# Wenlin-Chen/ADKF-IFT

Hardware: AMD Instinct MI355X
Metric: meta-tasks/sec (N_support=128, d=256) (higher is better)
Workload: dtype f32

## Files before the change

### adkf_ift_amd/csrc/adkf_gp.hip

```cpp
#include <hip/hip_runtime.h>
#include <algorithm>
#include <cstdio>
#include <cstdlib>

#include "../../include/adkf_gp.h"
#include "ard.h"
#include "pna.h"
#include "readout.h"
#include "block.h"
#include "outer_step.h"
#include "refine64.h"
#include "hyper.h"
#include "large_fused.h"
#include "gemm_x3.h"
#include "dense_x3.h"
#include "predict_stream.h"
#include "thompson_stream.h"

using namespace adkf;

namespace {

constexpr int MAX_POINTS = 4096;
constexpr int REG_POINTS = 128;
// ... 362 lines not shown

Refine64Args refine_args(const TaskView& tv, const adkf_batch_t* b, const Workspace& w, bool with_hessian, int level, float* f_out,
                         int32_t* info, float* f_in, float* g_in, float* gnorm, size_t& lds_bytes) {
    const bool lds_inv = refine64_lds_optin();
    lds_bytes = lds_inv ? sizeof(double) * (size_t)R64_LDS_POINTS * R64_LDS_POINTS : 0;
    return Refine64Args{tv, b->Z_s, b->Z_q, b->d, b->y_s, b->y_q, b->priors, w.Ainv, with_hessian ? w.P : nullptr, level >= 1 ? w.C : nullptr,
                        level >= 2 ? w.S : nullptr, w.vecs, w.scal, f_out, info, f_in, g_in, gnorm, w.w64, w.w64_stride, r64_threshold(), b->T,
                        with_hessian ? 1 : 0, level, lds_inv ? 1 : 0};
}

void launch_refine(const TaskView& tv, const adkf_batch_t* b, const Workspace& w, bool with_hessian, int level, float* f_out,
                   int32_t* info, hipStream_t st, float* f_in = nullptr, float* g_in = nullptr, float* gnorm = nullptr) {
    if (!w.w64) return;
    size_t lds_bytes;
    const Refine64Args ra = refine_args(tv, b, w, with_hessian, level, f_out, info, f_in, g_in, gnorm, lds_bytes);
    k_refine64<<<b->T, R64_NT, lds_bytes, st>>>(ra);
}

bool use_fused_outer(int ns, int nq) {
    static const bool enabled = [] { const char* e = getenv("ADKF_FUSED_OUTER"); return !e || atoi(e) != 0; }();
    static const bool optin = [] {
        bool ok = true;
        for (const void* f : {reinterpret_cast<const void*>(&k_hyper<true, 0>), reinterpret_cast<const void*>(&k_hyper<true, 1>),
                              reinterpret_cast<const void*>(&k_hyper<false, 0>), reinterpret_cast<const void*>(&k_hyper<false, 1>)})
            ok = ok && hipFuncSetAttribute(f, hipFuncAttributeMaxDynamicSharedMemorySize, (int)HY_LDS_BYTES) == hipSuccess;
        return ok;
    }();
    if (!optin) (void)hipGetLastError();
    const int hi = ns > nq ? ns : nq;
    return enabled && optin && hi >= 1 && hi <= HY_N;
}

int launch_outer_factor(const OuterArgs& a, const Workspace& w, int nq, hipStream_t st) {
    if (nq > REG_POINTS) {
        k_lg_resid<<<dim3(ceil_div(nq, 4), a.T), 256, 0, st>>>(a);
        LgMat m = lg_mat(w, a.S, a.tv.nq_ld, a.tv.n_q, nullptr, a.T);
        lg_sweep(m, st);
        LgMatvecArgs mv{m, a.vecs + (size_t)V_R * a.tv.vld, (size_t)NVEC * a.tv.vld, a.vecs + (size_t)V_E * a.tv.vld, (size_t)NVEC * a.tv.vld, -1.f};
        k_lg_matvec<<<dim3(ceil_div(nq, 4), a.T), 256, 0, st>>>(mv);
        const int tn = ceil_div(nq, GT);
        k_lg_negate<<<grid_for(a.T, tn * tn), 256, 0, st>>>(m, tn);
        LgColsumArgs cs{a.C, a.tv.ns_ld, (size_t)a.tv.nq_ld * a.tv.ns_ld, a.tv.n_q, a.tv.nq_ld, a.tv.n_s, a.tv.ns_ld,
                        a.vecs + (size_t)V_E * a.tv.vld, (size_t)NVEC * a.tv.vld, a.vecs + (size_t)V_CTE * a.tv.vld, (size_t)NVEC * a.tv.vld};
        k_lg_colsum<<<dim3(ceil_div(a.tv.ns_ld, 64), a.T), 1024, 0, st>>>(cs);
        LgOuterFin fin{a, w.lg_logdet, w.lg_info, w.lg_pext};
        k_lg_outer_fin<<<a.T, 64, 0, st>>>(fin);
        LAUNCH_OK();
        return 0;
    }
    if (nq <= 16) k_outer_factor<16, 256><<<grid_for(a.T, 1), 256, 0, st>>>(a);
    else if (nq <= 32) k_outer_factor<32, 256><<<grid_for(a.T, 1), 256, 0, st>>>(a);
    else if (nq <= 64) k_outer_factor<64, 256><<<grid_for(a.T, 1), 256, 0, st>>>(a);
    else k_outer_factor<128, 512><<<grid_for(a.T, 1), 512, 0, st>>>(a);
    LAUNCH_OK();
    return 0;
}


InnerArgs inner_args(const adkf_batch_t* b, const Workspace& w, float* phi, int32_t* info) {
    InnerArgs a{};
    a.D2ss = w.D2ss; a.y_s = b->y_s; a.n_s = b->n_s; a.phi = phi; a.priors = b->priors;
    a.Ainv = w.Ainv; a.vecs = w.vecs; a.scal = w.scal; a.info = info;
    a.T = b->T; a.ld = b->ns_max; a.vld = w.vld; a.kind = b->kernel;
    a.max_evals = 0; a.exact_evals = 0; a.gtol = 0.f; a.ftol = 0.f;
    return a;
}

int outer_pipeline(const adkf_batch_t* b, const Workspace& w, const float* phi, int flags, bool with_hessian, float* f_out,
                   float* dZ_s, float* dZ_q, float* g_phi_out, float* v_out, float* H_out, int32_t* info, hipStream_t st) {
    const int T = b->T, ns = b->ns_max, nq = b->nq_max, d = b->d;
    int rc = stage_dist(b, w, true, st);
    if (rc) return rc;
    const bool reuse_inner = (b->flags & ADKF_BATCH_REUSE_INNER) != 0;
    if (!reuse_inner) {
        InnerArgs ia = inner_args(b, w, const_cast<float*>(phi), info);
        rc = launch_inner(ia, w, st);
        if (rc) return rc;
    }
    TaskView tv = make_tv(b, w, true);
    const int tms = ceil_div(ns, GT), tmq = ceil_div(nq, GT);
    const float dirscale = (flags & ADKF_IGNORE_DIRECT_GRAD) ? 0.f : 1.f;
    const float corrscale = (with_hessian && !(flags & ADKF_IGNORE_GRAD_CORRECTION)) ? 1.f : 0.f;
    if (use_fused_outer(ns, nq)) {
        HyperArgs ha{tv, w.Ainv, w.D2ss, w.D2qs, w.D2qq, b->y_s, b->y_q, b->priors, w.Wss, w.Wqs, w.Wqq, w.P, w.OC, w.S, w.vecs, w.scal, f_out, info,
                     g_phi_out, v_out, H_out, T, reuse_inner ? 1 : 0, with_hessian ? 1 : 0, flags, dirscale, corrscale, refine32_threshold()};
        const bool full = ns == HY_N && nq == HY_N && !b->n_s && !b->n_q && tv.vec;
        const bool rbf = b->kernel == ADKF_KERNEL_RBF;
        if (full && rbf) k_hyper<true, 0><<<grid_for(T, 1), HY_NT, HY_LDS_BYTES, st>>>(ha);
        else if (full) k_hyper<true, 1><<<grid_for(T, 1), HY_NT, HY_LDS_BYTES, st>>>(ha);
        else if (rbf) k_hyper<false, 0><<<grid_for(T, 1), HY_NT, HY_LDS_BYTES, st>>>(ha);
        else k_hyper<false, 1><<<grid_for(T, 1), HY_NT, HY_LDS_BYTES, st>>>(ha);
    } else {
    launch_alpha_refine(tv, b, w, st);
    if (with_hessian) {
        ProbP pp; pp.tv = tv; pp.Ainv = w.Ainv; pp.D2ss = w.D2ss; pp.P = w.P;
        launch_gemm(pp, T, ns, ns, st);
        HessArgs ha{tv, w.Ainv, w.P, w.D2ss, b->y_s, b->priors, w.scal, w.vecs, T};
        if (ns > REG_POINTS) {
            k_lg_hess_mv<<<dim3(ceil_div(ns, 4), T), 256, 0, st>>>(ha);
            LgMat am = lg_mat(w, w.Ainv, ns, b->n_s, nullptr, T);
            LgMatvecArgs mv{am, w.vecs + (size_t)V_BETA * w.vld, (size_t)NVEC * w.vld, w.vecs + (size_t)V_DELTA * w.vld, (size_t)NVEC * w.vld, 1.f};
            k_lg_matvec<<<dim3(ceil_div(ns, 4), T), 256, 0, st>>>(mv);
            LgHessTr ht{ha, w.lg_part, tms * tms, tms};
            k_lg_hess_tr<<<grid_for(T, tms * tms), 256, 0, st>>>(ht);
            k_lg_hess_fin<<<T, 64, 0, st>>>(ht);
        } else {
            k_hess<<<grid_for(T, 1), SMALL_NT, 0, st>>>(ha);
        }
    }
    launch_c(tv, b, w, st);
    ProbS ps; ps.tv = tv; ps.C = w.C; ps.D2qs = w.D2qs; ps.D2qq = w.D2qq; ps.S = w.S;
    launch_gemm(ps, T, nq, nq, st);
    OuterArgs oa{tv, w.C, w.S, b->y_s, b->y_q, w.vecs, w.scal, f_out, info, T, reuse_inner ? 1 : 0};
    rc = launch_outer_factor(oa, w, nq, st);
    if (rc) return rc;
    ProbOC po; po.tv = tv; po.Sinv = w.S; po.C = w.C; po.D2qs = w.D2qs; po.OC = w.OC; po.Wqs = w.Wqs; po.part = w.part_oc; po.ntiles = w.nt_oc; po.dirscale = dirscale;
    launch_gemm(po, T, nq, ns, st);
    ProbMA pm; pm.tv = tv; pm.C = w.C; pm.OC = w.OC; pm.D2ss = w.D2ss; pm.Wss = w.Wss; pm.part = w.part_ma; pm.ntiles = w.nt_ma; pm.dirscale = dirscale;
    launch_gemm(pm, T, ns, ns, st);
    SolveArgs sa{tv, w.scal, w.vecs, w.part_oc, w.part_ma, w.nt_oc, w.nt_ma, flags, g_phi_out, v_out, H_out, T, with_hessian ? 1 : 0};
    WqqArgs wq{tv, w.S, w.D2qq, w.Wqq, w.scal, dirscale, T, 0, sa};
    if (nq > REG_POINTS) {
        LgWqq lw{wq, w.lg_part, tmq * tmq, tmq};
        k_lg_wqq<<<grid_for(T, tmq * tmq), 256, 0, st>>>(lw);
        k_lg_wqq_fin<<<T, 64, 0, st>>>(lw);
        k_solve_v<<<T, 64, 0, st>>>(sa);
    } else {
        wq.do_solve = 1;
        k_wqq<<<grid_for(T, 1), SMALL_NT, 0, st>>>(wq);
    }
    if (corrscale != 0.f) {
        ProbMixed px; px.tv = tv; px.Ainv = w.Ainv; px.P = w.P; px.D2ss = w.D2ss; px.Wss = w.Wss; px.corrscale = corrscale;
        launch_gemm(px, T, ns, ns, st);
    }
    }
    if (dZ_s || dZ_q) {
        if (dZ_s && b->n_s) hipMemsetAsync(dZ_s, 0, (size_t)T * ns * d * sizeof(float), st);
        if (dZ_q && b->n_q) hipMemsetAsync(dZ_q, 0, (size_t)T * nq * d * sizeof(float), st);
        ProbDZ<false> pzs; pzs.tv = tv; pzs.Wss = w.Wss; pzs.Wqs = w.Wqs; pzs.Wqq = w.Wqq; pzs.Zs = b->Z_s; pzs.Zq = b->Z_q; pzs.dZ = dZ_s; pzs.d = d;
        ProbDZ<true> pzq; pzq.tv = tv; pzq.Wss = w.Wss; pzq.Wqs = w.Wqs; pzq.Wqq = w.Wqq; pzq.Zs = b->Z_s; pzq.Zq = b->Z_q; pzq.dZ = dZ_q; pzq.d = d;
        if (dZ_s) launch_gemm(pzs, T, ns, d, st, x3_for(d));
        if (dZ_q) launch_gemm(pzq, T, nq, d, st, x3_for(d));
    }
    if (w.w64) {
        size_t lds_bytes;
        const Refine64Args ra = refine_args(tv, b, w, with_hessian, 2, f_out, info, nullptr, nullptr, nullptr, lds_bytes);
        Cot64Args ca{tv, b->Z_s, b->Z_q, dZ_s, dZ_q, d, w.vecs, w.scal, w.w64, w.w64_stride, r64_threshold(), T,
                     with_hessian ? 1 : 0, flags, dirscale, corrscale, g_phi_out, v_out, H_out, lds_bytes ? 1 : 0};
        k_tail64<<<T, R64_NT, lds_bytes, st>>>(ra, ca);
    }
    LAUNCH_OK();
    return 0;
}


struct ArdWs {
    float *mu, *ell, *Zt_s, *Zt_q, *G, *Gd_s, *Gd_q, *Gdot, *phi3, *pri3, *f3, *g3, *g3o, *S1, *gt, *coldot;
    float *c, *ut2, *wn, *Ddot, *Wdot, *adot, *S2;
    ArdFitState* fst; float *x, *g, *p, *xe, *ge, *S, *Y, *fe; int32_t* info3;
    ArdCgState* cst; float *cx, *cr, *cp, *cHp, *gout; int32_t* n_eff;
    size_t bytes;
};

ArdWs carve_ard(void* base, size_t off0, int T, int ns, int nq, int d) {
    ArdWs a;
    size_t off = off0;
    auto take = [&](size_t nfloat) { float* p = base ? reinterpret_cast<float*>(static_cast<char*>(base) + off) : nullptr; off += align_up((nfloat ? nfloat : 1) * sizeof(float)); return p; };
// ... 1208 lines not shown
```

### adkf_ift_amd/csrc/hyper.h

```cpp
#pragma once
#include "kernels.h"

namespace adkf {

constexpr int HY_NT = 512, HY_N = 128;
constexpr int HY_LDK = 132;
constexpr int HY_LDM = 144;
constexpr int HY_BUF = HY_N * HY_LDM;
constexpr int HY_NVEC = 10;
constexpr int HY_LDS_FLOATS = 2 * HY_BUF + HY_NVEC * HY_N + 9 * (HY_NT / 64) + 8;
constexpr size_t HY_LDS_BYTES = sizeof(float) * HY_LDS_FLOATS;

struct HyperArgs {
    TaskView tv;
    const float *Ainv, *D2ss, *D2qs, *D2qq, *y_s, *y_q, *priors;
    float *Wss, *Wqs, *Wqq;
    float *stash_ss, *stash_qs, *stash_qq;
    float* vecs; float* scal; float* f_out; int32_t* info;
    float *g_phi_out, *v_out, *H_out;
    int T, reset_info, with_hessian, flags;
    float dirscale, corrscale, refine_thresh;
};

__device__ __forceinline__ float hy_ex(int kind, float u) { return kind == 0 ? expf(-0.5f * u) : expf(-SQRT5 * sqrtf(u)); }
__device__ __forceinline__ float hy_k0(int kind, float u, float ex) { return kind == 0 ? ex : (1.f + SQRT5 * sqrtf(u) + (5.f / 3.f) * u) * ex; }
__device__ __forceinline__ float hy_ex_of_k0(int kind, float u, float k0) { return kind == 0 ? k0 : k0 / (1.f + SQRT5 * sqrtf(u) + (5.f / 3.f) * u); }
__device__ __forceinline__ void hy_k3(int kind, float u, float ex, float& k0, float& k1, float& k2) {
    if (kind == 0) { k0 = ex; k1 = -0.5f * ex; k2 = 0.25f * ex; }
    else {
        const float r = sqrtf(u);
        k0 = (1.f + SQRT5 * r + (5.f / 3.f) * u) * ex;
        k1 = -(5.f / 6.f) * (1.f + SQRT5 * r) * ex;
        k2 = (25.f / 12.f) * ex;
    }
}

#define HY_OPAQUE1(v_) asm volatile("" : "+v"(v_))
__device__ __forceinline__ int hy_tid() { int t = threadIdx.x; HY_OPAQUE1(t); return t; }
template <bool FULL>
__device__ __forceinline__ void hy_fetch(float4 (&v)[8], const float* src, int src_ld, int rows) {
    const int tid = threadIdx.x;
    unsigned base = (unsigned)((tid >> 5) * HY_N + (tid & 31) * 4);
    if (FULL) HY_OPAQUE1(base);
#pragma unroll
    for (int u = 0; u < 8; ++u) {
        const int r = (tid >> 5) + 16 * u, c4 = (tid & 31) * 4;
        if (FULL) v[u] = *reinterpret_cast<const float4*>(src + (base + 16u * u * HY_N));
        else {
            const int rc = r < rows ? r : rows - 1, cc = c4 + 3 < src_ld ? c4 : 0;
            v[u] = *reinterpret_cast<const float4*>(src + (unsigned)(rc * src_ld + cc));
        }
    }
}
template <bool FULL, class F>
__device__ __forceinline__ void hy_put(float* buf, int ld, const float4 (&v)[8], int rows, int cols, F f) {
    const int tid = hy_tid();
#pragma unroll
    for (int u = 0; u < 8; ++u) {
        const int r = (tid >> 5) + 16 * u, c4 = (tid & 31) * 4;
        float4 o;
        o.x = (FULL || (r < rows && c4 + 0 < cols)) ? f(v[u].x, r, c4 + 0) : 0.f;
        o.y = (FULL || (r < rows && c4 + 1 < cols)) ? f(v[u].y, r, c4 + 1) : 0.f;
        o.z = (FULL || (r < rows && c4 + 2 < cols)) ? f(v[u].z, r, c4 + 2) : 0.f;
        o.w = (FULL || (r < rows && c4 + 3 < cols)) ? f(v[u].w, r, c4 + 3) : 0.f;
        *reinterpret_cast<float4*>(buf + r * ld + c4) = o;
    }
}
template <bool FULL, class F>
__device__ __forceinline__ void hy_load(float* buf, int ld, const float* src, int src_ld, int rows, int cols, bool vec, F f) {
    if (FULL || vec) {
        float4 v[8];
        hy_fetch<FULL>(v, src, src_ld, rows);
        hy_put<FULL>(buf, ld, v, rows, cols, f);
    } else {
        for (int e = threadIdx.x; e < HY_N * HY_N; e += HY_NT) {
            const int r = e >> 7, c = e & 127;
            buf[r * ld + c] = (r < rows && c < cols) ? f(src[(unsigned)(r * src_ld + c)], r, c) : 0.f;
        }
    }
}

template <bool FULL, bool SYM>
__device__ __forceinline__ void hy_dist(float (&dv)[8][4], const float* D, int ld, int rows, int cols) {
    const int lane = threadIdx.x & 63, p = lane & 15, g = lane >> 4, w = threadIdx.x >> 6;
    if (FULL && SYM) {
        unsigned q = (unsigned)(p * HY_N + 16 * w + 4 * g);
        HY_OPAQUE1(q);
#pragma unroll
        for (int x = 0; x < 8; ++x) {
            const float4 t = *reinterpret_cast<const float4*>(D + (q + 16u * x * HY_N));
            dv[x][0] = t.x; dv[x][1] = t.y; dv[x][2] = t.z; dv[x][3] = t.w;
        }
    } else if (FULL) {
        unsigned q = (unsigned)((16 * w + 4 * g) * HY_N + p);
        HY_OPAQUE1(q);
#pragma unroll
        for (int x = 0; x < 8; ++x)
#pragma unroll
            for (int y = 0; y < 4; ++y) dv[x][y] = D[q + (unsigned)(y * HY_N + 16 * x)];
    } else {
        unsigned ro[4];
#pragma unroll
        for (int y = 0; y < 4; ++y) ro[y] = (unsigned)(min(16 * w + 4 * g + y, rows - 1) * ld);
#pragma unroll
        for (int x = 0; x < 8; ++x) {
            const unsigned co = (unsigned)min(16 * x + p, cols - 1);
#pragma unroll
            for (int y = 0; y < 4; ++y) dv[x][y] = D[ro[y] + co];
        }
// ... 6 lines not shown
    float b[8][4];
    __device__ __forceinline__ void fetch(const float* ap, int lda, const float* bp, int ldb, int kb) {
        if (A_MN) {
#pragma unroll
            for (int j = 0; j < 4; ++j) a[j] = ap[(16 * kb + j) * lda];
        } else {
            const float4 t = *reinterpret_cast<const float4*>(ap + 16 * kb);
            a[0] = t.x; a[1] = t.y; a[2] = t.z; a[3] = t.w;
        }
#pragma unroll
        for (int x = 0; x < 8; ++x) {
            if (B_MN) {
#pragma unroll
                for (int j = 0; j < 4; ++j) b[x][j] = bp[(16 * kb + j) * ldb + 16 * x];
            } else {
                const float4 t = *reinterpret_cast<const float4*>(bp + 16 * x * ldb + 16 * kb);
                b[x][0] = t.x; b[x][1] = t.y; b[x][2] = t.z; b[x][3] = t.w;
            }
        }
    }
    __device__ __forceinline__ void multiply(f32x4_t (&acc)[8]) const {
#pragma unroll
        for (int j = 0; j < 4; ++j)
#pragma unroll
            for (int x = 0; x < 8; ++x) acc[x] = __builtin_amdgcn_mfma_f32_16x16x4f32(a[j], b[x][j], acc[x], 0, 0, 0);
    }
};

template <bool A_MN, bool B_MN, bool DB = true>
__device__ __forceinline__ void hy_gemm(f32x4_t (&acc)[8], const float* A, int lda, const float* B, int ldb, int kblocks) {
    const int tid = hy_tid(), lane = tid & 63, p = lane & 15, g = lane >> 4, w = tid >> 6;
    const float* ap = A_MN ? A + (4 * g) * lda + 16 * w + p : A + (16 * w + p) * lda + 4 * g;
    const float* bp = B_MN ? B + (4 * g) * ldb + p : B + p * ldb + 4 * g;
    if constexpr (!DB) {
#pragma unroll 1
        for (int kb = 0; kb < kblocks; ++kb) {
            HyFrag<A_MN, B_MN> f;
            f.fetch(ap, lda, bp, ldb, kb);
            f.multiply(acc);
        }
    } else {
        HyFrag<A_MN, B_MN> f0, f1;
        f0.fetch(ap, lda, bp, ldb, 0);
        int kb = 0;
#pragma unroll 1
        for (; kb + 2 <= kblocks; kb += 2) {
            f1.fetch(ap, lda, bp, ldb, kb + 1);
            f0.multiply(acc);
            if (kb + 2 < kblocks) f0.fetch(ap, lda, bp, ldb, kb + 2);
            f1.multiply(acc);
        }
        if (kb < kblocks) f0.multiply(acc);
    }
}

__device__ __forceinline__ void hy_zero(f32x4_t (&acc)[8]) {
#pragma unroll
    for (int x = 0; x < 8; ++x) acc[x] = (f32x4_t){0.f, 0.f, 0.f, 0.f};
}

__device__ __forceinline__ void hy_store_t(const f32x4_t (&acc)[8], float* buf, int ld, float sign = 1.f) {
    const int tid = hy_tid(), lane = tid & 63, p = lane & 15, g = lane >> 4, w = tid >> 6;
#pragma unroll
    for (int x = 0; x < 8; ++x)
        *reinterpret_cast<float4*>(buf + (16 * x + p) * ld + 16 * w + 4 * g) =
            make_float4(sign * acc[x][0], sign * acc[x][1], sign * acc[x][2], sign * acc[x][3]);
}

__device__ __forceinline__ void hy_sym_store(float* G, const float (&v)[8][4]) {
    const int lane = threadIdx.x & 63, p = lane & 15, g = lane >> 4, w = threadIdx.x >> 6;
    unsigned q = (unsigned)(p * HY_N + 16 * w + 4 * g);
    HY_OPAQUE1(q);
#pragma unroll
    for (int x = 0; x < 8; ++x) *reinterpret_cast<float4*>(G + (q + 16u * x * HY_N)) = make_float4(v[x][0], v[x][1], v[x][2], v[x][3]);
}
__device__ __forceinline__ unsigned hy_sym_offset() {
    const int lane = threadIdx.x & 63, p = lane & 15, g = lane >> 4, w = threadIdx.x >> 6;
    unsigned q = (unsigned)(p * HY_N + 16 * w + 4 * g);
    HY_OPAQUE1(q);
    return q;
}
__device__ __forceinline__ void hy_sym_store_tile(float* G, unsigned q, int x, const float (&v)[4]) {
    *reinterpret_cast<float4*>(G + (q + 16u * x * HY_N)) = make_float4(v[0], v[1], v[2], v[3]);
}
__device__ __forceinline__ void hy_sym_load(float (&v)[8][4], const float* G) {
    const int lane = threadIdx.x & 63, p = lane & 15, g = lane >> 4, w = threadIdx.x >> 6;
    unsigned q = (unsigned)(p * HY_N + 16 * w + 4 * g);
    HY_OPAQUE1(q);
#pragma unroll
    for (int x = 0; x < 8; ++x) {
        const float4 t = *reinterpret_cast<const float4*>(G + (q + 16u * x * HY_N));
        v[x][0] = t.x; v[x][1] = t.y; v[x][2] = t.z; v[x][3] = t.w;
    }
}

template <int K>
__device__ __forceinline__ void hy_sum(const float (&v)[K], float* part, double* out) {
    const int tid = hy_tid(), lane = tid & 63, w = tid >> 6;
#pragma unroll
    for (int q = 0; q < K; ++q) {
        float s = v[q];
        s += dpp_f<DPP_XOR1>(s); s += dpp_f<DPP_XOR2>(s); s += dpp_f<DPP_HALF_MIRROR>(s); s += dpp_f<DPP_MIRROR>(s);
        if ((lane & 15) == 0) part[q * 32 + w * 4 + (lane >> 4)] = s;
    }
    __syncthreads();
    if (tid < K) {
        double s = 0.0;
#pragma unroll
        for (int i = 0; i < 8; ++i) {
            const float4 t = *reinterpret_cast<const float4*>(part + tid * 32 + 4 * i);
            s += ((double)t.x + (double)t.y) + ((double)t.z + (double)t.w);
        }
        out[tid] = s;
    }
    __syncthreads();
}

template <bool TWO>
__device__ __forceinline__ void hy_colsum(const float* M, int ld, const float* M2, int ld2, int rows, const float* x, float* scratch, float* out, float* out2) {
    const int tid = hy_tid(), j = tid & 127, part = tid >> 7;
    const int per = (rows + 3) >> 2, i0 = part * per, i1 = min(rows, i0 + per);
    float s0 = 0.f, s1 = 0.f, t0 = 0.f, t1 = 0.f;
    int i = i0;
    for (; i + 2 <= i1; i += 2) {
        const float x0 = x[i], x1 = x[i + 1];
        s0 = fmaf(M[i * ld + j], x0, s0); s1 = fmaf(M[(i + 1) * ld + j], x1, s1);
        if (TWO) { t0 = fmaf(M2[i * ld2 + j], x0, t0); t1 = fmaf(M2[(i + 1) * ld2 + j], x1, t1); }
    }
    if (i < i1) { s0 = fmaf(M[i * ld + j], x[i], s0); if (TWO) t0 = fmaf(M2[i * ld2 + j], x[i], t0); }
    scratch[tid] = s0 + s1;
    if (TWO) scratch[512 + tid] = t0 + t1;
    __syncthreads();
    if (tid < 128) out[tid] = (scratch[tid] + scratch[128 + tid]) + (scratch[256 + tid] + scratch[384 + tid]);
    else if (TWO && tid < 256) out2[tid - 128] = (scratch[512 + tid - 128] + scratch[512 + tid]) + (scratch[512 + 128 + tid] + scratch[512 + 256 + tid]);
    __syncthreads();
}

#define HY_FENCE() __builtin_amdgcn_sched_barrier(0)
#define HY_OPAQUE4(v_) asm volatile("" : "+v"((v_)[0]), "+v"((v_)[1]), "+v"((v_)[2]), "+v"((v_)[3]))
#define HY_OPAQUE3(a_, b_, c_) asm volatile("" : "+v"(a_), "+v"(b_), "+v"(c_))
#define HY_OPAQUE2(a_, b_) asm volatile("" : "+v"(a_), "+v"(b_))

template <bool FULL, int KIND>
__global__ __launch_bounds__(HY_NT, 1) void k_hyper(HyperArgs a) {
    using SW = Sweep<128, 512>;
    __shared__ SweepSmem<128, 512> sm;
    extern __shared__ __align__(16) float hy_lds[];
    int t, tile;
    if (!task_tile(a.T, 1, t, tile)) return;
    const int tid = threadIdx.x, lane = tid & 63, p = lane & 15, g = lane >> 4, w = tid >> 6;
    const int n = FULL ? HY_N : a.tv.ns(t), m = FULL ? HY_N : a.tv.nq(t), lds = FULL ? HY_N : a.tv.ns_ld, ldq = FULL ? HY_N : a.tv.nq_ld;
    const int vld = a.tv.vld;
    if (n <= 0 || m <= 0) return;
    float* X = hy_lds;
    float* Y = X + HY_BUF;
    float* al = Y + HY_BUF;
    float* ysv = al + HY_N;
    float* rv = ysv + HY_N;
    float* ev = rv + HY_N;
    float* cte = ev + HY_N;
    float* be = cte + HY_N;
    float* ga = be + HY_N;
    float* de = ga + HY_N;
    float* wv = de + HY_N;
    float* tmp = wv + HY_N;
    float* red = tmp + HY_N;
    float* bc = red + 9 * (HY_NT / 64);
    double* dsum = reinterpret_cast<double*>(red);
    float* scratch = sm.scratch();

    float* sc = a.scal + (size_t)t * NSCAL;
    const float noise = sc[S_NOISE], os = sc[S_OS], ls = sc[S_LS], il2 = 1.f / (ls * ls), gl = -2.f / ls;
    constexpr int kind = KIND;
    const bool vec = FULL || a.tv.vec;
    const float* Ai = a.Ainv + (size_t)t * lds * lds;
    const float* Dss = a.D2ss + (size_t)t * lds * lds;
    const float* Dqs = a.D2qs + (size_t)t * ldq * lds;
    const float* Dqq = a.D2qq + (size_t)t * ldq * ldq;
    float* st_ss = a.stash_ss + (size_t)t * HY_N * HY_N;
    float* st_qs = a.stash_qs + (size_t)t * HY_N * HY_N;
    float* st_qq = a.stash_qq + (size_t)t * HY_N * HY_N;
    float* vb = a.vecs + (size_t)t * NVEC * vld;
    const int kn = FULL ? 8 : (n + 15) >> 4, km = FULL ? 8 : (m + 15) >> 4;
    const bool refine = sc[S_CONDA] > a.refine_thresh;
    const bool refine_alpha = refine && sc[S_AREF] == 0.f;
    const int i0 = 16 * w + 4 * g, j0 = p;
    auto in_s = [&](int i) { return FULL || i < n; };
    auto in_q = [&](int i) { return FULL || i < m; };

    if (tid < HY_N) {
        al[tid] = tid < n ? vb[V_ALPHA * vld + tid] : 0.f;
        ysv[tid] = tid < n ? a.y_s[(size_t)t * lds + tid] : 0.f;
        rv[tid] = tid < m ? a.y_q[(size_t)t * ldq + tid] : 0.f;
    }
    auto ident = [](float v, int, int) { return v; };
    auto k0fun = [=](float d2, int, int) { const float u = d2 * il2; return os * hy_k0(kind, u, hy_ex(kind, u)); };
    auto afun = [=](float d2, int r, int c) { const float u = d2 * il2; return os * hy_k0(kind, u, hy_ex(kind, u)) + (r == c ? noise : 0.f); };

    {
        float4 va[8], vk[8];
        hy_fetch<FULL>(va, Ai, lds, n);
        hy_fetch<FULL>(vk, Dqs, lds, m);
        if (FULL || vec) {
            hy_put<FULL>(Y, HY_LDK, va, n, n, ident);
            hy_put<FULL>(X, HY_LDK, vk, m, n, k0fun);
        }
        if (FULL) {
#pragma unroll
            for (int u = 0; u < 8; ++u) {
                const int r = (tid >> 5) + 16 * u, c4 = (tid & 31) * 4;
                *reinterpret_cast<float4*>(st_qs + (unsigned)(r * HY_N + c4)) = *reinterpret_cast<const float4*>(X + r * HY_LDK + c4);
            }
        }
    }
    if (!(FULL || vec)) {
        hy_load<false>(Y, HY_LDK, Ai, lds, n, n, false, ident);
        hy_load<false>(X, HY_LDK, Dqs, lds, m, n, false, k0fun);
    }
    __syncthreads();
    f32x4_t acc[8];
    hy_zero(acc);
    hy_gemm<false, false>(acc, Y, HY_LDK, X, HY_LDK, kn);
    if (refine) {
        __syncthreads();
        hy_store_t(acc, Y, HY_LDM);
        hy_load<FULL>(X, HY_LDK, Dss, lds, n, n, vec, afun);
        __syncthreads();
        if (refine_alpha) {
            hy_colsum<false>(X, HY_LDK, nullptr, 0, n, al, scratch, tmp, nullptr);
            if (tid < HY_N) tmp[tid] = tid < n ? ysv[tid] - tmp[tid] : 0.f;
        }
        f32x4_t rr[8];
        hy_zero(rr);
        hy_gemm<false, false>(rr, X, HY_LDK, Y, HY_LDM, kn);
#pragma unroll
        for (int x = 0; x < 8; ++x) {
#pragma unroll
            for (int y = 0; y < 4; ++y) {
                const int i = i0 + y, j = j0 + 16 * x;
                const float u = Dqs[(unsigned)(min(j, m - 1) * lds + min(i, n - 1))] * il2;
                rr[x][y] = (i < n && j < m) ? os * hy_k0(kind, u, hy_ex(kind, u)) - rr[x][y] : 0.f;
            }
            HY_OPAQUE4(rr[x]);
            HY_FENCE();
        }
        __syncthreads();
        hy_store_t(rr, Y, HY_LDK);
        hy_load<FULL>(X, HY_LDK, Ai, lds, n, n, vec, ident);
        __syncthreads();
        if (refine_alpha) {
            hy_colsum<false>(X, HY_LDK, nullptr, 0, n, tmp, scratch, be, nullptr);
            if (tid < n) { al[tid] += be[tid]; vb[V_ALPHA * vld + tid] = al[tid]; }
            if (tid == 0) sc[S_AREF] = 1.f;
        }
        hy_gemm<false, false>(acc, X, HY_LDK, Y, HY_LDK, kn);
        __syncthreads();
        hy_load<FULL>(X, HY_LDK, Dqs, lds, m, n, vec, k0fun);
    }
    __syncthreads();
    hy_store_t(acc, Y, HY_LDM);
    __syncthreads();

    {
        const int i = tid >> 2, q = tid & 3;
        float s = 0.f;
#pragma unroll
        for (int u = 0; u < 8; ++u) {
            const int k = 16 * u + 4 * q;
            const float4 c4 = *reinterpret_cast<const float4*>(Y + i * HY_LDM + k);
            const float4 y4 = *reinterpret_cast<const float4*>(ysv + k);
            s = fmaf(c4.x, y4.x, fmaf(c4.y, y4.y, fmaf(c4.z, y4.z, fmaf(c4.w, y4.w, s))));
        }
        s += dpp_f<DPP_XOR1>(s);
        s += dpp_f<DPP_XOR2>(s);
        if (q == 0) {
            sm.vec_in[i] = i < m ? rv[i] - s : 0.f;
            if (i < m) vb[V_MU * vld + i] = s;
        }
    }
    hy_zero(acc);
    hy_gemm<false, false>(acc, Y, HY_LDM, X, HY_LDK, kn);
    float mm[8][4];
    {
        float dv[8][4];
        hy_dist<FULL, true>(dv, Dqq, ldq, m, m);
        const unsigned sq = hy_sym_offset();
#pragma unroll
        for (int x = 0; x < 8; ++x) {
            float eqq[4];
#pragma unroll
            for (int y = 0; y < 4; ++y) {
                const int i = i0 + y, j = j0 + 16 * x;
                const float u = dv[x][y] * il2;
                eqq[y] = hy_ex(kind, u);
                const float sv = os * hy_k0(kind, u, eqq[y]) + (i == j ? noise : 0.f) - acc[x][y];
                mm[x][y] = (in_q(i) && in_q(j)) ? sv : (i == j ? 1.f : 0.f);
            }
            if (FULL) hy_sym_store_tile(st_qq, sq, x, eqq);
            HY_OPAQUE4(mm[x]);
            HY_FENCE();
        }
    }
    __syncthreads();
    SW::run(mm, m, sm);
    float logdet;
    const int info = SW::finish(m, sm, logdet);
    const float pivr = pivot_ratio<HY_NT>(sm.pivs, m, sm.red);
    SW::solve(mm, sm.vec_in, sm.vec_out);
    float qv[1] = {0.f};
    if (tid < HY_N) {
        const float e = tid < m ? sm.vec_out[tid] : 0.f, r = tid < m ? sm.vec_in[tid] : 0.f;
        ev[tid] = e;
        if (tid < m) { vb[V_E * vld + tid] = e; vb[V_R * vld + tid] = r; }
        qv[0] = r * e;
    }
    block_sum<1, HY_NT>(qv, red);
    const float fval = 0.5f * qv[0] + 0.5f * logdet + 0.5f * (float)m * LOG_2PI;
    if (tid == 0) {
        sc[S_PIVR_S] = pivr; sc[S_FOUT] = fval; sc[S_LOGDETS] = logdet;
        if (a.f_out) a.f_out[t] = (info == 0) ? fval : NAN;
        if (a.reset_info) a.info[t] = info != 0 ? 100000 + info : 0;
        else if (info != 0 && a.info[t] == 0) a.info[t] = 100000 + info;
    }
    float r8[9] = {0.f, 0.f, 0.f, 0.f, 0.f, 0.f, 0.f, 0.f, 0.f};
    auto rows_cols = [&](const float* vsrc, float (&vi)[4], float (&vj)[8]) {
#pragma unroll
        for (int y = 0; y < 4; ++y) vi[y] = vsrc[i0 + y];
#pragma unroll
        for (int x = 0; x < 8; ++x) vj[x] = vsrc[j0 + 16 * x];
    };
    {
        float e_i[4], e_j[8];
        rows_cols(ev, e_i, e_j);
        f32x4_t si[8];
#pragma unroll
        for (int x = 0; x < 8; ++x) si[x] = (f32x4_t){mm[x][0], mm[x][1], mm[x][2], mm[x][3]};
        hy_store_t(si, X, HY_LDK, -1.f);
        float* Wo = a.Wqq + (size_t)t * ldq * ldq;
        float dv[8][4], eqq[8][4];
        hy_dist<FULL, true>(dv, Dqq, ldq, m, m);
        if (FULL) hy_sym_load(eqq, st_qq);
        const float wsc = a.dirscale * os * il2;
        const unsigned sq = hy_sym_offset();
#pragma unroll
        for (int x = 0; x < 8; ++x) {
            float wq[4];
#pragma unroll
            for (int y = 0; y < 4; ++y) {
                const int i = i0 + y, j = j0 + 16 * x;
                wq[y] = 0.f;
                if (in_q(i) && in_q(j)) {
                    const float om = 0.5f * (-mm[x][y] - e_i[y] * e_j[x]);
                    float k0, k1, k2; const float u = dv[x][y] * il2; hy_k3(kind, u, FULL ? eqq[x][y] : hy_ex(kind, u), k0, k1, k2);
                    wq[y] = wsc * om * k1;
                    if (!FULL) Wo[(unsigned)(i * ldq + j)] = wq[y];
                    if (i == j) r8[0] += om;
                    r8[1] += om * k0;
                    r8[2] += om * os * k1 * u * gl;
                }
            }
            if (FULL) hy_sym_store_tile(Wo, sq, x, wq);
            HY_OPAQUE3(r8[0], r8[1], r8[2]);
            HY_FENCE();
        }
    }
    hy_colsum<false>(Y, HY_LDM, nullptr, 0, m, ev, scratch, cte, nullptr);
    if (tid < n) vb[V_CTE * vld + tid] = cte[tid];
    hy_zero(acc);
    hy_gemm<false, true>(acc, X, HY_LDK, Y, HY_LDM, km);
    {
        float* Wo = a.Wqs + (size_t)t * ldq * lds;
        float e_i[4], e_j[8], al_i[4], al_j[8], cte_i[4], cte_j[8];
        rows_cols(ev, e_i, e_j);
        rows_cols(al, al_i, al_j);
        rows_cols(cte, cte_i, cte_j);
        float dv[8][4], kq[8][4];
        hy_dist<FULL, false>(dv, Dqs, lds, m, n);
        if (FULL) hy_dist<true, false>(kq, st_qs, HY_N, HY_N, HY_N);
        const float wsc = a.dirscale * os * il2;
#pragma unroll
        for (int x = 0; x < 8; ++x) {
#pragma unroll
            for (int y = 0; y < 4; ++y) {
                const int i = i0 + y, j = j0 + 16 * x;
                float oc = 0.f;
                if (in_q(i) && in_s(j)) {
                    oc = 0.5f * (acc[x][y] - e_i[y] * cte_j[x]);
                    const float MB = -2.f * oc - e_i[y] * al_j[x];
                    float k0, k1, k2; const float u = dv[x][y] * il2;
                    hy_k3(kind, u, FULL ? hy_ex_of_k0(kind, u, kq[x][y] / os) : hy_ex(kind, u), k0, k1, k2);
                    Wo[(unsigned)(i * lds + j)] = wsc * MB * k1;
                    r8[3] += MB * k0;
                    r8[4] += MB * os * k1 * u * gl;
                }
                acc[x][y] = oc;
            }
            HY_OPAQUE2(r8[3], r8[4]); HY_OPAQUE4(acc[x]);
            HY_FENCE();
        }
    }
    __syncthreads();
    hy_store_t(acc, X, HY_LDK);
    __syncthreads();
    hy_zero(acc);
    hy_gemm<true, false>(acc, Y, HY_LDM, X, HY_LDK, km);
    float* Wss_o = a.Wss + (size_t)t * lds * lds;
    {
        float al_i[4], al_j[8], cte_i[4], cte_j[8];
        rows_cols(al, al_i, al_j);
        rows_cols(cte, cte_i, cte_j);
        float dv[8][4];
        hy_dist<FULL, true>(dv, Dss, lds, n, n);
        const float wsc = a.dirscale * os * il2;
        const unsigned sq = hy_sym_offset();
#pragma unroll
        for (int x = 0; x < 8; ++x) {
            float ess[4], wss[4];
#pragma unroll
            for (int y = 0; y < 4; ++y) {
                const int i = i0 + y, j = j0 + 16 * x;
                wss[y] = 0.f; ess[y] = 0.f;
                float gv = 0.f;
                if (in_s(i) && in_s(j)) {
                    const float MA = acc[x][y] + 0.5f * (cte_i[y] * al_j[x] + al_i[y] * cte_j[x]);
                    const float u = dv[x][y] * il2;
                    ess[y] = hy_ex(kind, u);
                    float k0, k1, k2; hy_k3(kind, u, ess[y], k0, k1, k2);
                    wss[y] = wsc * MA * k1;
                    if (!FULL) Wss_o[(unsigned)(i * lds + j)] = wss[y];
                    gv = os * k1 * u * gl;
                    if (i == j) r8[5] += MA;
                    r8[6] += MA * k0;
                    r8[7] += MA * gv;
                }
                acc[x][y] = gv;
            }
            if (FULL) { hy_sym_store_tile(Wss_o, sq, x, wss); hy_sym_store_tile(st_ss, sq, x, ess); }
            HY_OPAQUE3(r8[5], r8[6], r8[7]); HY_OPAQUE4(acc[x]);
            HY_FENCE();
        }
    }
    hy_sum<9>(r8, scratch, dsum);
    const float d1n = sc[S_D1N], d1s = sc[S_D1S], d1l = sc[S_D1L];
    const float g0 = (float)(dsum[0] + dsum[5]) * d1n;
    const float g1 = (float)(dsum[6] + dsum[3] + dsum[1]) * d1s;
    const float g2 = (float)(dsum[7] + dsum[4] + dsum[2]) * d1l;
    if (tid == 0) {
        sc[S_QQ_TR] = (float)dsum[0]; sc[S_QQ_K] = (float)dsum[1]; sc[S_QQ_L] = (float)dsum[2];
        sc[S_GOUT0] = g0; sc[S_GOUT1] = g1; sc[S_GOUT2] = g2;
        if (a.g_phi_out) { a.g_phi_out[t * 3 + 0] = g0; a.g_phi_out[t * 3 + 1] = g1; a.g_phi_out[t * 3 + 2] = g2; }
    }
    __syncthreads();

    float cn = 0.f, cs = 0.f, cl = 0.f;
    if (a.with_hessian) {
        hy_load<FULL>(Y, HY_LDK, Ai, lds, n, n, vec, ident);
        hy_store_t(acc, X, HY_LDK);
        __syncthreads();
        hy_colsum<true>(X, HY_LDK, Y, HY_LDK, n, al, scratch, be, ga);
        hy_colsum<false>(Y, HY_LDK, nullptr, 0, n, be, scratch, de, nullptr);
        if (tid < n) { vb[V_BETA * vld + tid] = be[tid]; vb[V_GAMMA * vld + tid] = ga[tid]; vb[V_DELTA * vld + tid] = de[tid]; }
        hy_zero(acc);
        hy_gemm<false, false>(acc, Y, HY_LDK, X, HY_LDK, kn);
        float h9[9] = {0.f, 0.f, 0.f, 0.f, 0.f, 0.f, 0.f, 0.f, 0.f};
        {
            float al_i[4], al_j[8];
            rows_cols(al, al_i, al_j);
            float dv[8][4], ess[8][4];
            hy_dist<FULL, true>(dv, Dss, lds, n, n);
            if (FULL) hy_sym_load(ess, st_ss);
#pragma unroll
            for (int x = 0; x < 8; ++x) {
#pragma unroll
                for (int y = 0; y < 4; ++y) {
                    const int i = i0 + y, j = j0 + 16 * x;
                    if (in_s(i) && in_s(j)) {
                        const float ai = Y[i * HY_LDK + j];
                        float k0, k1, k2; const float u = dv[x][y] * il2; hy_k3(kind, u, FULL ? ess[x][y] : hy_ex(kind, u), k0, k1, k2);
                        const float Kll = os * (k2 * 4.f * u * u + k1 * 6.f * u) * il2;
                        h9[0] += ai * ai; h9[1] += acc[x][y] * ai; h9[3] += ai * Kll; h9[4] += al_i[y] * al_j[x] * Kll;
                    }
                }
                HY_OPAQUE2(h9[0], h9[1]); HY_OPAQUE2(h9[3], h9[4]);
                HY_FENCE();
            }
        }
        __syncthreads();
        hy_store_t(acc, X, HY_LDK);
        __syncthreads();
#pragma unroll
        for (int x = 0; x < 8; ++x) {
#pragma unroll
            for (int y = 0; y < 4; ++y) {
                const int i = i0 + y, j = j0 + 16 * x;
                if (in_s(i) && in_s(j)) h9[2] += acc[x][y] * X[i * HY_LDK + j];
            }
            asm volatile("" : "+v"(h9[2]));
            HY_FENCE();
        }
        if (tid < n) { h9[5] = al[tid] * ga[tid]; h9[6] = be[tid] * ga[tid]; h9[7] = be[tid] * de[tid]; h9[8] = al[tid] * be[tid]; }
        hy_sum<9>(h9, scratch, dsum);
        if (tid == 0) {
#pragma unroll
            for (int q = 0; q < 9; ++q) h9[q] = (float)dsum[q];
            hess_assemble(sc, a.priors + t * 4, n, h9);
            float v[3] = {0.f, 0.f, 0.f};
            if (!(a.flags & 1)) {
                double Mx[3][4];
                const float gg[3] = {g0, g1, g2};
                for (int i = 0; i < 3; ++i) { for (int j = 0; j < 3; ++j) Mx[i][j] = sc[S_H0 + i * 3 + j]; Mx[i][3] = gg[i]; }
                for (int c = 0; c < 3; ++c) {
                    int pv = c;
                    for (int r = c + 1; r < 3; ++r) if (fabs(Mx[r][c]) > fabs(Mx[pv][c])) pv = r;
                    if (pv != c) for (int j = 0; j < 4; ++j) { const double tm = Mx[c][j]; Mx[c][j] = Mx[pv][j]; Mx[pv][j] = tm; }
                    const double ip = 1.0 / Mx[c][c];
                    for (int r = c + 1; r < 3; ++r) { const double f = Mx[r][c] * ip; for (int j = c; j < 4; ++j) Mx[r][j] -= f * Mx[c][j]; }
                }
                double vd[3] = {0.0, 0.0, 0.0};
                for (int c = 2; c >= 0; --c) { double s = Mx[c][3]; for (int j = c + 1; j < 3; ++j) s -= Mx[c][j] * vd[j]; vd[c] = s / Mx[c][c]; }
                for (int c = 0; c < 3; ++c) v[c] = (float)vd[c];
            }
            sc[S_V0] = v[0]; sc[S_V1] = v[1]; sc[S_V2] = v[2];
            const float cn_ = v[0] * d1n, cs_ = v[1] * d1s / os, cl_ = v[2] * d1l;
            sc[S_CN] = cn_; sc[S_CS] = cs_; sc[S_CL] = cl_;
            bc[0] = cn_; bc[1] = cs_; bc[2] = cl_;
            if (a.v_out) { a.v_out[t * 3 + 0] = v[0]; a.v_out[t * 3 + 1] = v[1]; a.v_out[t * 3 + 2] = v[2]; }
            if (a.H_out) for (int q = 0; q < 9; ++q) a.H_out[t * 9 + q] = sc[S_H0 + q];
        }
        __syncthreads();
        cn = bc[0]; cs = bc[1]; cl = bc[2];
        if (tid < HY_N) {
            const float wval = tid < n ? cn * ga[tid] + cs * (al[tid] - noise * ga[tid]) + cl * de[tid] : 0.f;
            wv[tid] = wval;
            if (tid < n) vb[V_W * vld + tid] = wval;
        }
        if (a.corrscale != 0.f) {
            const float ca = cn - cs * noise;
            const int tb = hy_tid();
#pragma unroll
            for (int u = 0; u < 8; ++u) {
                const int r = (tb >> 5) + 16 * u, c4 = (tb & 31) * 4;
                float4 xv = *reinterpret_cast<float4*>(X + r * HY_LDK + c4);
                const float4 yv = *reinterpret_cast<const float4*>(Y + r * HY_LDK + c4);
                xv.x = cl * xv.x + ca * yv.x + ((r == c4 + 0 && r < n) ? cs : 0.f);
                xv.y = cl * xv.y + ca * yv.y + ((r == c4 + 1 && r < n) ? cs : 0.f);
                xv.z = cl * xv.z + ca * yv.z + ((r == c4 + 2 && r < n) ? cs : 0.f);
                xv.w = cl * xv.w + ca * yv.w + ((r == c4 + 3 && r < n) ? cs : 0.f);
                *reinterpret_cast<float4*>(X + r * HY_LDK + c4) = xv;
            }
            __syncthreads();
            hy_zero(acc);
            hy_gemm<true, false>(acc, X, HY_LDK, Y, HY_LDK, kn);
            float dv[8][4], ess[8][4], wss[8][4];
            hy_dist<FULL, true>(dv, Dss, lds, n, n);
            if (FULL) { hy_sym_load(ess, st_ss); hy_sym_load(wss, Wss_o); }
            const float ifn = 1.f / (float)n;
            const unsigned sq = hy_sym_offset();
            float w_i[4], w_j[8], al_i[4], al_j[8];
            rows_cols(wv, w_i, w_j);
            rows_cols(al, al_i, al_j);
#pragma unroll
            for (int x = 0; x < 8; ++x) {
#pragma unroll
                for (int y = 0; y < 4; ++y) {
                    const int i = i0 + y, j = j0 + 16 * x;
                    if (in_s(i) && in_s(j)) {
                        const float dgdA = (-0.5f * acc[x][y] + 0.5f * (w_i[y] * al_j[x] + al_i[y] * w_j[x])) * ifn;
                        const float Q = 0.5f * (Y[i * HY_LDK + j] - al_i[y] * al_j[x]) * ifn;
                        float k0, k1, k2; const float u = dv[x][y] * il2; hy_k3(kind, u, FULL ? ess[x][y] : hy_ex(kind, u), k0, k1, k2);
                        const float dBv = cs * os * k1 + cl * os * gl * (k1 + u * k2);
                        const float corr = a.corrscale * (dgdA * os * k1 * il2 + Q * dBv * il2);
                        if (FULL) wss[x][y] -= corr;
                        else Wss_o[(unsigned)(i * lds + j)] -= corr;
                    }
                }
                if (FULL) hy_sym_store_tile(Wss_o, sq, x, wss[x]);
                HY_FENCE();
            }
        }
    } else if (tid == 0) {
        sc[S_V0] = sc[S_V1] = sc[S_V2] = 0.f;
        sc[S_CN] = sc[S_CS] = sc[S_CL] = 0.f;
        if (a.v_out) { a.v_out[t * 3 + 0] = 0.f; a.v_out[t * 3 + 1] = 0.f; a.v_out[t * 3 + 2] = 0.f; }
        if (a.H_out) for (int q = 0; q < 9; ++q) a.H_out[t * 9 + q] = 0.f;
    }
}

}
```

Baseline: 282,600.

## Keep kernel exponentials and distances in registers instead of global stash buffers

Removes the global-memory stash buffers (stash_ss/qs/qq) in the fused hyper kernel. The exp terms, squared distances and Wss tiles are now kept in per-thread register arrays across phases, and the Wss store is deferred when the gradient correction will rewrite it. The query-support exponentials are recomputed rather than recovered from the stashed kernel values. This removes global round-trips and repeated distance loads, at the cost of much higher register pressure, which may reduce occupancy or cause spills.

Result: faster. 290,900, median of 6 (+2.9%).

```diff
diff --git a/adkf_ift_amd/csrc/adkf_gp.hip b/adkf_ift_amd/csrc/adkf_gp.hip
--- a/adkf_ift_amd/csrc/adkf_gp.hip
+++ b/adkf_ift_amd/csrc/adkf_gp.hip
@@ -468,7 +468,7 @@
     const float dirscale = (flags & ADKF_IGNORE_DIRECT_GRAD) ? 0.f : 1.f;
     const float corrscale = (with_hessian && !(flags & ADKF_IGNORE_GRAD_CORRECTION)) ? 1.f : 0.f;
     if (use_fused_outer(ns, nq)) {
-        HyperArgs ha{tv, w.Ainv, w.D2ss, w.D2qs, w.D2qq, b->y_s, b->y_q, b->priors, w.Wss, w.Wqs, w.Wqq, w.P, w.OC, w.S, w.vecs, w.scal, f_out, info,
+        HyperArgs ha{tv, w.Ainv, w.D2ss, w.D2qs, w.D2qq, b->y_s, b->y_q, b->priors, w.Wss, w.Wqs, w.Wqq, w.vecs, w.scal, f_out, info,
                      g_phi_out, v_out, H_out, T, reuse_inner ? 1 : 0, with_hessian ? 1 : 0, flags, dirscale, corrscale, refine32_threshold()};
         const bool full = ns == HY_N && nq == HY_N && !b->n_s && !b->n_q && tv.vec;
         const bool rbf = b->kernel == ADKF_KERNEL_RBF;
diff --git a/adkf_ift_amd/csrc/hyper.h b/adkf_ift_amd/csrc/hyper.h
--- a/adkf_ift_amd/csrc/hyper.h
+++ b/adkf_ift_amd/csrc/hyper.h
@@ -15,7 +15,6 @@
     TaskView tv;
     const float *Ainv, *D2ss, *D2qs, *D2qq, *y_s, *y_q, *priors;
     float *Wss, *Wqs, *Wqq;
-    float *stash_ss, *stash_qs, *stash_qq;
     float* vecs; float* scal; float* f_out; int32_t* info;
     float *g_phi_out, *v_out, *H_out;
     int T, reset_info, with_hessian, flags;
@@ -24,7 +23,6 @@
 
 __device__ __forceinline__ float hy_ex(int kind, float u) { return kind == 0 ? expf(-0.5f * u) : expf(-SQRT5 * sqrtf(u)); }
 __device__ __forceinline__ float hy_k0(int kind, float u, float ex) { return kind == 0 ? ex : (1.f + SQRT5 * sqrtf(u) + (5.f / 3.f) * u) * ex; }
-__device__ __forceinline__ float hy_ex_of_k0(int kind, float u, float k0) { return kind == 0 ? k0 : k0 / (1.f + SQRT5 * sqrtf(u) + (5.f / 3.f) * u); }
 __device__ __forceinline__ void hy_k3(int kind, float u, float ex, float& k0, float& k1, float& k2) {
     if (kind == 0) { k0 = ex; k1 = -0.5f * ex; k2 = 0.25f * ex; }
     else {
@@ -197,16 +195,6 @@
 }
 __device__ __forceinline__ void hy_sym_store_tile(float* G, unsigned q, int x, const float (&v)[4]) {
     *reinterpret_cast<float4*>(G + (q + 16u * x * HY_N)) = make_float4(v[0], v[1], v[2], v[3]);
-}
-__device__ __forceinline__ void hy_sym_load(float (&v)[8][4], const float* G) {
-    const int lane = threadIdx.x & 63, p = lane & 15, g = lane >> 4, w = threadIdx.x >> 6;
-    unsigned q = (unsigned)(p * HY_N + 16 * w + 4 * g);
-    HY_OPAQUE1(q);
-#pragma unroll
-    for (int x = 0; x < 8; ++x) {
-        const float4 t = *reinterpret_cast<const float4*>(G + (q + 16u * x * HY_N));
-        v[x][0] = t.x; v[x][1] = t.y; v[x][2] = t.z; v[x][3] = t.w;
-    }
 }
 
 template <int K>
@@ -287,14 +275,12 @@
     float* sc = a.scal + (size_t)t * NSCAL;
     const float noise = sc[S_NOISE], os = sc[S_OS], ls = sc[S_LS], il2 = 1.f / (ls * ls), gl = -2.f / ls;
     constexpr int kind = KIND;
+    constexpr bool KEEP_DSS = FULL && KIND == 0;
     const bool vec = FULL || a.tv.vec;
     const float* Ai = a.Ainv + (size_t)t * lds * lds;
     const float* Dss = a.D2ss + (size_t)t * lds * lds;
     const float* Dqs = a.D2qs + (size_t)t * ldq * lds;
     const float* Dqq = a.D2qq + (size_t)t * ldq * ldq;
-    float* st_ss = a.stash_ss + (size_t)t * HY_N * HY_N;
-    float* st_qs = a.stash_qs + (size_t)t * HY_N * HY_N;
-    float* st_qq = a.stash_qq + (size_t)t * HY_N * HY_N;
     float* vb = a.vecs + (size_t)t * NVEC * vld;
     const int kn = FULL ? 8 : (n + 15) >> 4, km = FULL ? 8 : (m + 15) >> 4;
     const bool refine = sc[S_CONDA] > a.refine_thresh;
@@ -320,13 +306,6 @@
             hy_put<FULL>(Y, HY_LDK, va, n, n, ident);
             hy_put<FULL>(X, HY_LDK, vk, m, n, k0fun);
         }
-        if (FULL) {
-#pragma unroll
-            for (int u = 0; u < 8; ++u) {
-                const int r = (tid >> 5) + 16 * u, c4 = (tid & 31) * 4;
-                *reinterpret_cast<float4*>(st_qs + (unsigned)(r * HY_N + c4)) = *reinterpret_cast<const float4*>(X + r * HY_LDK + c4);
-            }
-        }
     }
     if (!(FULL || vec)) {
         hy_load<false>(Y, HY_LDK, Ai, lds, n, n, false, ident);
@@ -396,23 +375,21 @@
     hy_zero(acc);
     hy_gemm<false, false>(acc, Y, HY_LDM, X, HY_LDK, kn);
     float mm[8][4];
+    float dqq[8][4], eqq[8][4];
     {
-        float dv[8][4];
-        hy_dist<FULL, true>(dv, Dqq, ldq, m, m);
-        const unsigned sq = hy_sym_offset();
-#pragma unroll
-        for (int x = 0; x < 8; ++x) {
-            float eqq[4];
+        hy_dist<FULL, true>(dqq, Dqq, ldq, m, m);
+#pragma unroll
+        for (int x = 0; x < 8; ++x) {
 #pragma unroll
             for (int y = 0; y < 4; ++y) {
                 const int i = i0 + y, j = j0 + 16 * x;
-                const float u = dv[x][y] * il2;
-                eqq[y] = hy_ex(kind, u);
-                const float sv = os * hy_k0(kind, u, eqq[y]) + (i == j ? noise : 0.f) - acc[x][y];
+                const float u = dqq[x][y] * il2;
+                eqq[x][y] = hy_ex(kind, u);
+                const float sv = os * hy_k0(kind, u, eqq[x][y]) + (i == j ? noise : 0.f) - acc[x][y];
                 mm[x][y] = (in_q(i) && in_q(j)) ? sv : (i == j ? 1.f : 0.f);
             }
-            if (FULL) hy_sym_store_tile(st_qq, sq, x, eqq);
             HY_OPAQUE4(mm[x]);
+            if (FULL) HY_OPAQUE4(eqq[x]);
             HY_FENCE();
         }
     }
@@ -452,9 +429,7 @@
         for (int x = 0; x < 8; ++x) si[x] = (f32x4_t){mm[x][0], mm[x][1], mm[x][2], mm[x][3]};
         hy_store_t(si, X, HY_LDK, -1.f);
         float* Wo = a.Wqq + (size_t)t * ldq * ldq;
-        float dv[8][4], eqq[8][4];
-        hy_dist<FULL, true>(dv, Dqq, ldq, m, m);
-        if (FULL) hy_sym_load(eqq, st_qq);
+        if (!FULL) hy_dist<FULL, true>(dqq, Dqq, ldq, m, m);
         const float wsc = a.dirscale * os * il2;
         const unsigned sq = hy_sym_offset();
 #pragma unroll
@@ -466,7 +441,7 @@
                 wq[y] = 0.f;
                 if (in_q(i) && in_q(j)) {
                     const float om = 0.5f * (-mm[x][y] - e_i[y] * e_j[x]);
-                    float k0, k1, k2; const float u = dv[x][y] * il2; hy_k3(kind, u, FULL ? eqq[x][y] : hy_ex(kind, u), k0, k1, k2);
+                    float k0, k1, k2; const float u = dqq[x][y] * il2; hy_k3(kind, u, FULL ? eqq[x][y] : hy_ex(kind, u), k0, k1, k2);
                     wq[y] = wsc * om * k1;
                     if (!FULL) Wo[(unsigned)(i * ldq + j)] = wq[y];
                     if (i == j) r8[0] += om;
@@ -489,9 +464,8 @@
         rows_cols(ev, e_i, e_j);
         rows_cols(al, al_i, al_j);
         rows_cols(cte, cte_i, cte_j);
-        float dv[8][4], kq[8][4];
+        float dv[8][4];
         hy_dist<FULL, false>(dv, Dqs, lds, m, n);
-        if (FULL) hy_dist<true, false>(kq, st_qs, HY_N, HY_N, HY_N);
         const float wsc = a.dirscale * os * il2;
 #pragma unroll
         for (int x = 0; x < 8; ++x) {
@@ -503,7 +477,7 @@
                     oc = 0.5f * (acc[x][y] - e_i[y] * cte_j[x]);
                     const float MB = -2.f * oc - e_i[y] * al_j[x];
                     float k0, k1, k2; const float u = dv[x][y] * il2;
-                    hy_k3(kind, u, FULL ? hy_ex_of_k0(kind, u, kq[x][y] / os) : hy_ex(kind, u), k0, k1, k2);
+                    hy_k3(kind, u, hy_ex(kind, u), k0, k1, k2);
                     Wo[(unsigned)(i * lds + j)] = wsc * MB * k1;
                     r8[3] += MB * k0;
                     r8[4] += MB * os * k1 * u * gl;
@@ -520,29 +494,29 @@
     hy_zero(acc);
     hy_gemm<true, false>(acc, Y, HY_LDM, X, HY_LDK, km);
     float* Wss_o = a.Wss + (size_t)t * lds * lds;
+    const bool defer_wss = FULL && a.with_hessian && a.corrscale != 0.f;
+    float dss[8][4], ess[8][4], wss[8][4];
     {
         float al_i[4], al_j[8], cte_i[4], cte_j[8];
         rows_cols(al, al_i, al_j);
         rows_cols(cte, cte_i, cte_j);
-        float dv[8][4];
-        hy_dist<FULL, true>(dv, Dss, lds, n, n);
+        hy_dist<FULL, true>(dss, Dss, lds, n, n);
         const float wsc = a.dirscale * os * il2;
         const unsigned sq = hy_sym_offset();
 #pragma unroll
         for (int x = 0; x < 8; ++x) {
-            float ess[4], wss[4];
 #pragma unroll
             for (int y = 0; y < 4; ++y) {
                 const int i = i0 + y, j = j0 + 16 * x;
-                wss[y] = 0.f; ess[y] = 0.f;
+                wss[x][y] = 0.f; ess[x][y] = 0.f;
                 float gv = 0.f;
                 if (in_s(i) && in_s(j)) {
                     const float MA = acc[x][y] + 0.5f * (cte_i[y] * al_j[x] + al_i[y] * cte_j[x]);
-                    const float u = dv[x][y] * il2;
-                    ess[y] = hy_ex(kind, u);
-                    float k0, k1, k2; hy_k3(kind, u, ess[y], k0, k1, k2);
-                    wss[y] = wsc * MA * k1;
-                    if (!FULL) Wss_o[(unsigned)(i * lds + j)] = wss[y];
+                    const float u = dss[x][y] * il2;
+                    ess[x][y] = hy_ex(kind, u);
+                    float k0, k1, k2; hy_k3(kind, u, ess[x][y], k0, k1, k2);
+                    wss[x][y] = wsc * MA * k1;
+                    if (!FULL) Wss_o[(unsigned)(i * lds + j)] = wss[x][y];
                     gv = os * k1 * u * gl;
                     if (i == j) r8[5] += MA;
                     r8[6] += MA * k0;
@@ -550,7 +524,9 @@
                 }
                 acc[x][y] = gv;
             }
-            if (FULL) { hy_sym_store_tile(Wss_o, sq, x, wss); hy_sym_store_tile(st_ss, sq, x, ess); }
+            if (FULL && !defer_wss) hy_sym_store_tile(Wss_o, sq, x, wss[x]);
+            if (FULL) HY_OPAQUE4(ess[x]);
+            if (FULL) HY_OPAQUE4(wss[x]);
             HY_OPAQUE3(r8[5], r8[6], r8[7]); HY_OPAQUE4(acc[x]);
             HY_FENCE();
         }
@@ -581,9 +557,7 @@
         {
             float al_i[4], al_j[8];
             rows_cols(al, al_i, al_j);
-            float dv[8][4], ess[8][4];
-            hy_dist<FULL, true>(dv, Dss, lds, n, n);
-            if (FULL) hy_sym_load(ess, st_ss);
+            if (!KEEP_DSS) hy_dist<FULL, true>(dss, Dss, lds, n, n);
 #pragma unroll
             for (int x = 0; x < 8; ++x) {
 #pragma unroll
@@ -591,7 +565,7 @@
                     const int i = i0 + y, j = j0 + 16 * x;
                     if (in_s(i) && in_s(j)) {
                         const float ai = Y[i * HY_LDK + j];
-                        float k0, k1, k2; const float u = dv[x][y] * il2; hy_k3(kind, u, FULL ? ess[x][y] : hy_ex(kind, u), k0, k1, k2);
+                        float k0, k1, k2; const float u = dss[x][y] * il2; hy_k3(kind, u, FULL ? ess[x][y] : hy_ex(kind, u), k0, k1, k2);
                         const float Kll = os * (k2 * 4.f * u * u + k1 * 6.f * u) * il2;
                         h9[0] += ai * ai; h9[1] += acc[x][y] * ai; h9[3] += ai * Kll; h9[4] += al_i[y] * al_j[x] * Kll;
                     }
@@ -666,9 +640,7 @@
             __syncthreads();
             hy_zero(acc);
             hy_gemm<true, false>(acc, X, HY_LDK, Y, HY_LDK, kn);
-            float dv[8][4], ess[8][4], wss[8][4];
-            hy_dist<FULL, true>(dv, Dss, lds, n, n);
-            if (FULL) { hy_sym_load(ess, st_ss); hy_sym_load(wss, Wss_o); }
+            if (!KEEP_DSS) hy_dist<FULL, true>(dss, Dss, lds, n, n);
             const float ifn = 1.f / (float)n;
             const unsigned sq = hy_sym_offset();
             float w_i[4], w_j[8], al_i[4], al_j[8];
@@ -682,7 +654,7 @@
                     if (in_s(i) && in_s(j)) {
                         const float dgdA = (-0.5f * acc[x][y] + 0.5f * (w_i[y] * al_j[x] + al_i[y] * w_j[x])) * ifn;
                         const float Q = 0.5f * (Y[i * HY_LDK + j] - al_i[y] * al_j[x]) * ifn;
-                        float k0, k1, k2; const float u = dv[x][y] * il2; hy_k3(kind, u, FULL ? ess[x][y] : hy_ex(kind, u), k0, k1, k2);
+                        float k0, k1, k2; const float u = dss[x][y] * il2; hy_k3(kind, u, FULL ? ess[x][y] : hy_ex(kind, u), k0, k1, k2);
                         const float dBv = cs * os * k1 + cl * os * gl * (k1 + u * k2);
                         const float corr = a.corrscale * (dgdA * os * k1 * il2 + Q * dBv * il2);
                         if (FULL) wss[x][y] -= corr;
```
